# interestingLSY/swiftLLM

Measured on AMD Instinct MI355X. Metric: decode tok/s (llama3-8b bfloat16, batch 32/GPU, 1024-in/128-out; prefill tok/s alongside), higher is better.
Workload: dtype bf16

## Files before the change

swiftllm_amd/csrc/prefill_attn.hip:

```cpp
#include <stdlib.h>

#include "prefill_tile.h"

namespace swl {

struct PrefillParams {
    void *o;
    const void *q;
    const void *k;
    const void *v;
    const int *cu_seqlens;
    int num_seqs, H, KVH, num_q_blocks;
    int hpw;
    float scale_log2e;
    int64_t q_tok_stride, k_tok_stride, v_tok_stride, o_tok_stride;
};

template <typename T, int D>
__global__ __launch_bounds__(256, 2) void prefill_attn_kernel(PrefillParams p) {
    constexpr int KRS = D + 8;
    constexpr int VRS = D + 32;
    constexpr int KSTEPS = D / 16;
    constexpr int DT = D / 32;
    constexpr int CPR = D / 8;
    constexpr int RPP = 256 / CPR;
    constexpr int NPASS = kBK / RPP;
    __shared__ __attribute__((aligned(16))) T smem[kBK * KRS + kBK * VRS];
    T *const Ks = smem;
    T *const Vs = smem + kBK * KRS;

    const PrefillGrid u = PrefillGrid::decode(blockIdx.x, p.num_seqs, p.H, p.KVH, p.num_q_blocks, 1);
    if (!u.valid) return;
    const int kvh = u.kvh;
    const int head = kvh * (p.H / p.KVH) + u.hgroup;
    const int start = p.cu_seqlens[u.seq];
    const int len = p.cu_seqlens[u.seq + 1] - start;
    const int q0 = u.qb * kBQ;
    if (q0 >= len) return;

    const int tid = threadIdx.x;
    const int lane = tid & 63;
    const int wave = __builtin_amdgcn_readfirstlane(tid >> 6);
    const int l32 = lane & 31;
    const int hf = lane >> 5;
    const int q0w = q0 + wave * 32;
    const int qrow = q0w + l32;
    const float c = p.scale_log2e;

    const T *qg = static_cast<const T *>(p.q);
    const T *kg = static_cast<const T *>(p.k) + static_cast<int64_t>(kvh) * D;
    const T *vg = static_cast<const T *>(p.v) + static_cast<int64_t>(kvh) * D;

    vec8_t<T> qf[KSTEPS];
    prefill_load_q<T, D>(qf, qg, start, head, p.q_tok_stride, qrow, len, hf);

    float16_t ot[DT];
#pragma unroll
    for (int dt = 0; dt < DT; ++dt) ot[dt] = float16_t{};
    float m_run = kNegBig;
    float l_run = 0.f;

    const int srow = tid / CPR;
    const int sc = tid % CPR;
    vec8_t<T> kst[NPASS], vst[NPASS];
    const T *kp[NPASS], *vp[NPASS];
#pragma unroll
    for (int ps = 0; ps < NPASS; ++ps) {
        const int64_t tok = static_cast<int64_t>(start) + srow + ps * RPP;
        kp[ps] = kg + tok * p.k_tok_stride + sc * 8;
        vp[ps] = vg + tok * p.v_tok_stride + sc * 8;
    }
    const int64_t kstep = static_cast<int64_t>(kBK) * p.k_tok_stride, vstep = static_cast<int64_t>(kBK) * p.v_tok_stride;
    auto fetch_tile = [&](int key0) {
        if (key0 + kBK <= len) {
#pragma unroll
            for (int ps = 0; ps < NPASS; ++ps) {
                kst[ps] = load8(kp[ps]);
                vst[ps] = load8(vp[ps]);
            }
        } else {
#pragma unroll
            for (int ps = 0; ps < NPASS; ++ps) {
                vec8_t<T> kt = vec8_t<T>{}, vt = vec8_t<T>{};
                if (key0 + srow + ps * RPP < len) {
                    kt = load8(kp[ps]);
                    vt = load8(vp[ps]);
                }
                kst[ps] = kt;
                vst[ps] = vt;
            }
        }
#pragma unroll
        for (int ps = 0; ps < NPASS; ++ps) {
            kp[ps] += kstep;
            vp[ps] += vstep;
        }
    };
    auto commit_tile = [&]() {
#pragma unroll
        for (int ps = 0; ps < NPASS; ++ps) {
            const int r = srow + ps * RPP;
            *reinterpret_cast<vec8_t<T> *>(&Ks[r * KRS + sc * 8]) = kst[ps];
            *reinterpret_cast<vec8_t<T> *>(&Vs[r * VRS + sc * 8]) = vst[ps];
        }
    };

    const int kv_end = min(len, q0 + kBQ);
    const int ntiles = (kv_end + kBK - 1) / kBK;

    const int k_frag_off = l32 * KRS + hf * 8;
    const int i16 = lane & 15;
    const int v_frag_off = (4 * hf + (i16 >> 2)) * VRS + 16 * ((lane >> 4) & 1) + 4 * (i16 & 3);

    fetch_tile(0);
    for (int tile = 0; tile < ntiles; ++tile) {
        const int key0 = tile * kBK;
        __syncthreads();
        commit_tile();
        __syncthreads();
        if (tile + 1 < ntiles) fetch_tile(key0 + kBK);

        if (key0 > q0w + 31) continue;
        prefill_tile<T, D, true>(
            qf, ot, m_run, l_run, c, qrow - key0 - 4 * hf, key0 + kBK - 1 > q0w,
            [&](int t, int kk) { return *reinterpret_cast<const vec8_t<T> *>(&Ks[k_frag_off + t * 32 * KRS + kk * 16]); },
            [&](int t, int ks, int dt, int half) {
                return lds_tr_read(&Vs[v_frag_off + (t * 32 + 16 * ks + 8 * half) * VRS + dt * 32]);
            });
    }

    static_assert(4 * 32 * (D + 8) <= kBK * KRS + kBK * VRS, "the four waves' O tiles must fit the K/V tiles' LDS");
    __syncthreads();
    T *obase = static_cast<T *>(p.o) + static_cast<int64_t>(start) * p.o_tok_stride + static_cast<int64_t>(head) * D;
    prefill_store_rows<T, D, false>(ot, l_run, 1.0f, smem + wave * 32 * (D + 8), obase, p.o_tok_stride, q0w, len, lane, l32, hf);
}

__device__ __forceinline__ void dma_4_pieces(const unsigned (&off)[4], const char *base, unsigned lds) {
#pragma unroll
    for (int jj = 0; jj < 4; ++jj) {
        unsigned keep;
        asm volatile("s_mov_b32 %0, m0\n\ts_mov_b32 m0, %3\n\ts_nop 4\n\tglobal_load_lds_dwordx4 %1, %2\n\ts_mov_b32 m0, %0"
                     : "=&s"(keep) : "v"(off[jj]), "s"(base), "s"(lds + jj * 1024) : "memory");
    }
}

template <typename T>
__global__ __launch_bounds__(256, 2) void prefill_attn_dma_kernel(PrefillParams p) {
    constexpr int D = 128;
    constexpr int KSTEPS = D / 16, DT = D / 32;
    constexpr int ROWB = D * 2;
    constexpr int TILEB = kBK * ROWB;
    __shared__ __attribute__((aligned(16))) char smem[2 * 2 * TILEB];

    const int hpw = p.hpw;
    const int rows_wg = (4 / hpw) * 32;
    const PrefillGrid u = PrefillGrid::decode(blockIdx.x, p.num_seqs, p.H, p.KVH, p.num_q_blocks, hpw);
    if (!u.valid) return;
    const int kvh = u.kvh;
    const int start = p.cu_seqlens[u.seq];
    const int len = p.cu_seqlens[u.seq + 1] - start;
    const int q0 = u.qb * rows_wg;
    if (q0 >= len) return;

    const int tid = threadIdx.x;
    const int lane = tid & 63;
    const int wave = __builtin_amdgcn_readfirstlane(tid >> 6);
    const int head = kvh * (p.H / p.KVH) + u.hgroup * hpw + wave % hpw;
    const int l32 = lane & 31;
    const int hf = lane >> 5;
    const int q0w = q0 + (wave / hpw) * 32;
    const int qrow = q0w + l32;
    const float c = p.scale_log2e;

    const T *qg = static_cast<const T *>(p.q);
    vec8_t<T> qf[KSTEPS];

    float16_t ot[DT];
#pragma unroll
    for (int dt = 0; dt < DT; ++dt) ot[dt] = float16_t{};
    float m_run = kNegBig;
    float l_run = 0.f;

    const int drow = (lane >> 4);
    const int dslot = lane & 15;
    const unsigned lds0 = static_cast<unsigned>(reinterpret_cast<uintptr_t>(
        (__attribute__((address_space(3))) char *)smem));
    const int64_t kstride_b = p.k_tok_stride * 2, vstride_b = p.v_tok_stride * 2;
    unsigned koff[4], voff[4];
    auto dma_offsets = [&](int rows_valid) {
#pragma unroll
        for (int jj = 0; jj < 4; ++jj) {
            const int r = 16 * wave + 4 * jj + drow;
            const int rs = min(r, rows_valid - 1);
            koff[jj] = static_cast<unsigned>(rs * kstride_b) + static_cast<unsigned>((dslot ^ (r & 15)) * 16);
            voff[jj] = static_cast<unsigned>(rs * vstride_b) +
                       static_cast<unsigned>(((((dslot >> 2) ^ (r & 3)) << 2) | (dslot & 3)) * 16);
        }
    };
    dma_offsets(kBK);
    const char *kbase = reinterpret_cast<const char *>(static_cast<const T *>(p.k) + static_cast<int64_t>(kvh) * D) +
                        static_cast<int64_t>(start) * kstride_b;
    const char *vbase = reinterpret_cast<const char *>(static_cast<const T *>(p.v) + static_cast<int64_t>(kvh) * D) +
                        static_cast<int64_t>(start) * vstride_b;
    auto issue_tile = [&](int tile, int buf) {
        const char *kb = kbase + static_cast<int64_t>(tile) * kBK * kstride_b;
        const char *vb = vbase + static_cast<int64_t>(tile) * kBK * vstride_b;
        const unsigned ldsk = lds0 + static_cast<unsigned>(buf) * 2 * TILEB + static_cast<unsigned>(wave) * 4096;
        dma_4_pieces(koff, kb, ldsk);
        dma_4_pieces(voff, vb, ldsk + TILEB);
    };

    const int kv_end = min(len, q0 + rows_wg);
    const int ntiles = (kv_end + kBK - 1) / kBK;
    const int last_rows = kv_end - (ntiles - 1) * kBK > 0 ? min(kBK, len - (ntiles - 1) * kBK) : kBK;

    unsigned kfo[KSTEPS];
#pragma unroll
    for (int kk = 0; kk < KSTEPS; ++kk) kfo[kk] = static_cast<unsigned>(l32 * ROWB + (((2 * kk + hf) ^ (l32 & 15)) * 16));
    const int i16 = lane & 15;
    unsigned vfo[DT];
#pragma unroll
    for (int dt = 0; dt < DT; ++dt)
        vfo[dt] = static_cast<unsigned>(TILEB + (4 * hf + (i16 >> 2)) * ROWB + ((dt ^ ((i16 >> 2) & 3)) * 64) +
                                        32 * ((lane >> 4) & 1) + 8 * (i16 & 3));

    if (ntiles == 1 && last_rows < kBK) dma_offsets(last_rows);
    issue_tile(0, 0);
    {
        T *qs = reinterpret_cast<T *>(smem + 2 * TILEB) + wave * 32 * D;
        const int rsub = lane >> 4, pc = lane & 15;
        vec8_t<T> t[8];
#pragma unroll
        for (int i = 0; i < 8; ++i) {
            const int row = 4 * i + rsub;
            const bool ok = q0w + row < len;
            t[i] = load8(qg + (static_cast<int64_t>(start) + (ok ? q0w + row : 0)) * p.q_tok_stride +
                         static_cast<int64_t>(head) * D + pc * 8);
            if (!ok) t[i] = vec8_t<T>{};
        }
#pragma unroll
        for (int i = 0; i < 8; ++i) {
            const int row = 4 * i + rsub;
            *reinterpret_cast<vec8_t<T> *>(qs + row * D + ((pc ^ (row & 15)) << 3)) = t[i];
        }
#pragma unroll
        for (int kk = 0; kk < KSTEPS; ++kk)
            qf[kk] = *reinterpret_cast<const vec8_t<T> *>(qs + l32 * D + (((2 * kk + hf) ^ (l32 & 15)) << 3));
        asm volatile("s_waitcnt lgkmcnt(0)" ::: "memory");
    }
    for (int tile = 0; tile < ntiles; ++tile) {
        const int key0 = tile * kBK;
        const int buf = tile & 1;
        asm volatile("s_waitcnt vmcnt(0)" ::: "memory");
        __builtin_amdgcn_s_barrier();
        if (tile + 1 < ntiles) {
            if (tile + 2 == ntiles && last_rows < kBK) dma_offsets(last_rows);
            issue_tile(tile + 1, buf ^ 1);
        }
        if (key0 > q0w + 31) continue;
        const char *bufp = smem + buf * 2 * TILEB;
        prefill_tile<T, D, false>(
            qf, ot, m_run, l_run, c, qrow - key0 - 4 * hf, key0 + kBK - 1 > q0w,
            [&](int t, int kk) { return *reinterpret_cast<const vec8_t<T> *>(bufp + kfo[kk] + t * 32 * ROWB); },
            [&](int t, int ks, int dt, int half) {
                return lds_tr_read(reinterpret_cast<const T *>(bufp + vfo[dt] + (t * 32 + 16 * ks + 8 * half) * ROWB));
            });
    }

    static_assert(4 * 32 * (D + 8) * 2 <= 4 * TILEB, "the four waves' O tiles must fit the K/V buffers");
    __syncthreads();
    T *obase = static_cast<T *>(p.o) + static_cast<int64_t>(start) * p.o_tok_stride + static_cast<int64_t>(head) * D;
    prefill_store_rows<T, D, false>(ot, l_run, 1.0f, reinterpret_cast<T *>(smem) + wave * 32 * (D + 8), obase,
                                    p.o_tok_stride, q0w, len, lane, l32, hf);
}

}

extern "C" int swl_prefill_attn_varlen(void *o, const void *q, const void *k, const void *v,
                                       const int32_t *cu_seqlens, int32_t num_prefill_seqs,
                                       int32_t max_prefill_len, int32_t num_q_heads,
                                       int32_t num_kv_heads, int32_t head_dim, float softmax_scale,
                                       int64_t q_tok_stride, int64_t k_tok_stride,
                                       int64_t v_tok_stride, int64_t o_tok_stride, int32_t dtype,
                                       swl_stream_t stream) {
    if (num_prefill_seqs < 0 || max_prefill_len < 0) return SWL_ERR_BAD_ARG;
    if (num_prefill_seqs == 0 || max_prefill_len == 0) return SWL_OK;
    if (!o || !q || !k || !v || !cu_seqlens) return SWL_ERR_BAD_ARG;
    if (num_q_heads <= 0 || num_kv_heads <= 0 || num_q_heads % num_kv_heads != 0)
        return SWL_ERR_BAD_ARG;
    if (!(head_dim == 32 || head_dim == 64 || head_dim == 128)) return SWL_ERR_UNSUPPORTED;
    if ((q_tok_stride & 7) || (k_tok_stride & 7) || (v_tok_stride & 7) || (o_tok_stride & 7))
        return SWL_ERR_BAD_ARG;
    const int64_t q_row = static_cast<int64_t>(num_q_heads) * head_dim, kv_row = static_cast<int64_t>(num_kv_heads) * head_dim;
    if (q_tok_stride < q_row || o_tok_stride < q_row || k_tok_stride < kv_row || v_tok_stride < kv_row)
        return SWL_ERR_BAD_ARG;
    if (!swl::aligned16(q) || !swl::aligned16(k) || !swl::aligned16(v) || !swl::aligned16(o))
        return SWL_ERR_BAD_ARG;
    swl::PrefillParams p;
    p.o = o;
    p.q = q;
    p.k = k;
    p.v = v;
    p.cu_seqlens = cu_seqlens;
    p.num_seqs = num_prefill_seqs;
    p.H = num_q_heads;
    p.KVH = num_kv_heads;
    p.num_q_blocks = (max_prefill_len + swl::kBQ - 1) / swl::kBQ;
    p.scale_log2e = softmax_scale * 1.44269504088896340736f;
    p.q_tok_stride = q_tok_stride;
    p.k_tok_stride = k_tok_stride;
    p.v_tok_stride = v_tok_stride;
    p.o_tok_stride = o_tok_stride;
    p.hpw = 1;
    const int G = num_q_heads / num_kv_heads;
    dim3 grid;
    if (!swl::prefill_grid_blocks(num_prefill_seqs, num_kv_heads, G, p.num_q_blocks, &grid)) return SWL_ERR_UNSUPPORTED;
    hipStream_t s = static_cast<hipStream_t>(stream);
    static const bool use_v1 = [] { const char *e = getenv("SWL_PREFILL_ATTN"); return e && e[0] == 'v' && e[1] == '1'; }();
    const bool fits32 = static_cast<int64_t>(swl::kBK) * (k_tok_stride > v_tok_stride ? k_tok_stride : v_tok_stride) * 2 + 4096 < (1ll << 32);
    SWL_DISPATCH_DTYPE(dtype, T, {
        if (head_dim == 128 && !use_v1 && fits32) {
            static const int forced_hpw = [] { const char *e = getenv("SWL_PREFILL_HPW"); return e ? atoi(e) : 0; }();
            p.hpw = G % 2 == 0 ? 2 : 1;
            if (forced_hpw == 1 || forced_hpw == 2 || forced_hpw == 4) p.hpw = G % forced_hpw == 0 ? forced_hpw : p.hpw;
            const int rows_wg = (4 / p.hpw) * 32;
            p.num_q_blocks = (max_prefill_len + rows_wg - 1) / rows_wg;
            if (!swl::prefill_grid_blocks(num_prefill_seqs, num_kv_heads, G / p.hpw, p.num_q_blocks, &grid))
                return SWL_ERR_UNSUPPORTED;
            hipLaunchKernelGGL((swl::prefill_attn_dma_kernel<T>), grid, dim3(256), 0, s, p);
        }
        else if (head_dim == 128)
            hipLaunchKernelGGL((swl::prefill_attn_kernel<T, 128>), grid, dim3(256), 0, s, p);
        else if (head_dim == 64)
            hipLaunchKernelGGL((swl::prefill_attn_kernel<T, 64>), grid, dim3(256), 0, s, p);
        else
            hipLaunchKernelGGL((swl::prefill_attn_kernel<T, 32>), grid, dim3(256), 0, s, p);
    });
    return swl::check_launch();
}
```

swiftllm_amd/csrc/prefill_tile.h:

```cpp
#pragma once

#include "attn_mfma.h"

namespace swl {

constexpr int kBQ = 128;
constexpr int kBK = 64;

struct PrefillGrid {
    bool valid;
    int seq, kvh;
    int hgroup;
    int qb;
    static __device__ __forceinline__ PrefillGrid decode(int id, int num_seqs, int H, int KVH, int num_q_blocks, int hpw) {
        const int hgroups = H / KVH / hpw;
        const int per_unit = hgroups * num_q_blocks;
        const int xcd = id & 7;
        const int j = id >> 3;
        const int unit = xcd + 8 * (j / per_unit);
        const int inner = j % per_unit;
        return {unit < num_seqs * KVH, unit / KVH, unit % KVH, inner % hgroups, num_q_blocks - 1 - inner / hgroups};
    }
};

static inline bool prefill_grid_blocks(int num_seqs, int KVH, int hgroups, int num_q_blocks, dim3 *grid) {
    const int64_t units = static_cast<int64_t>(num_seqs) * KVH;
    const int64_t nblocks = (units + 7) / 8 * 8 * hgroups * num_q_blocks;
    if (nblocks > 0x7fffffffLL) return false;
    *grid = dim3(static_cast<unsigned>(nblocks));
    return true;
}

template <typename T, int D>
__device__ __forceinline__ void prefill_load_q(vec8_t<T> (&qf)[D / 16], const T *qg, int start, int head,
                                               int64_t q_tok_stride, int qrow, int len, int hf) {
    const bool ok = qrow < len;
    const T *qp = qg + (static_cast<int64_t>(start) + (ok ? qrow : 0)) * q_tok_stride + static_cast<int64_t>(head) * D + hf * 8;
#pragma unroll
    for (int kk = 0; kk < D / 16; ++kk) {
        vec8_t<T> t = load8(qp + kk * 16);
        if (!ok) t = vec8_t<T>{};
        qf[kk] = t;
    }
}

template <typename T, int D, bool PRIO, typename KFrag, typename VFrag>
__device__ __forceinline__ void prefill_tile(const vec8_t<T> (&qf)[D / 16], float16_t (&ot)[D / 32], float &m_run,
                                             float &l_run, float c, int dmask, bool diagonal, KFrag kfrag, VFrag vfrag) {
    constexpr int KSTEPS = D / 16, DT = D / 32;
    float16_t st[2];
    if constexpr (PRIO) __builtin_amdgcn_s_setprio(1);
#pragma unroll
    for (int t = 0; t < 2; ++t) {
        st[t] = float16_t{};
#pragma unroll
        for (int kk = 0; kk < KSTEPS; ++kk) {
            const vec8_t<T> kf = kfrag(t, kk);
            st[t] = mfma32(kf, qf[kk], st[t]);
        }
    }
    if constexpr (PRIO) __builtin_amdgcn_s_setprio(0);
    mfma_results_tie(st[0]);
    mfma_results_ready<8>(st[1]);
    if (diagonal) {
#pragma unroll
        for (int t = 0; t < 2; ++t)
#pragma unroll
            for (int r = 0; r < 16; ++r) {
                if ((r & 3) + 8 * (r >> 2) + t * 32 > dmask) st[t][r] = kNegBig;
            }
    }
    float mx = st[0][0];
#pragma unroll
    for (int t = 0; t < 2; ++t)
#pragma unroll
        for (int r = 0; r < 16; ++r) mx = fmaxf(mx, st[t][r]);
    mx = fmaxf(mx, __shfl_xor(mx, 32, 64));
    const float m_cand = fmaxf(m_run, mx * c);
    const float m_new = m_cand - m_run > kLazyMax ? m_cand : m_run;
    const float alpha = fast_exp2(m_run - m_new);
    m_run = m_new;
    float psum = 0.f;
#pragma unroll
    for (int t = 0; t < 2; ++t)
#pragma unroll
        for (int r = 0; r < 16; ++r) {
            const float pv = fast_exp2(fmaf(st[t][r], c, -m_new));
            st[t][r] = pv;
            psum += pv;
        }
    l_run = fmaf(l_run, alpha, psum);
    if (!__all(alpha == 1.0f)) {
#pragma unroll
        for (int dt = 0; dt < DT; ++dt)
#pragma unroll
            for (int r = 0; r < 16; ++r) ot[dt][r] *= alpha;
    }

    if constexpr (PRIO) __builtin_amdgcn_s_setprio(1);
#pragma unroll
    for (int t = 0; t < 2; ++t)
#pragma unroll
        for (int ks = 0; ks < 2; ++ks) {
            vec8_t<T> pb;
#pragma unroll
            for (int jj = 0; jj < 8; ++jj) pb[jj] = to_t<T>(st[t][8 * ks + jj]);
#pragma unroll
            for (int dt = 0; dt < DT; ++dt) {
                const short4_t lo = vfrag(t, ks, dt, 0);
                const short4_t hi = vfrag(t, ks, dt, 1);
                typedef short short8_t __attribute__((ext_vector_type(8)));
                const short8_t both = {lo[0], lo[1], lo[2], lo[3], hi[0], hi[1], hi[2], hi[3]};
                ot[dt] = mfma32(__builtin_bit_cast(vec8_t<T>, both), pb, ot[dt]);
            }
        }
    if constexpr (PRIO) __builtin_amdgcn_s_setprio(0);
}

template <typename T, int D, bool SCALED>
__device__ __forceinline__ void prefill_store_rows(float16_t (&ot)[D / 32], float l_run, float v_scale, T *ow, T *obase,
                                                   int64_t o_tok_stride, int q0w, int len, int lane, int l32, int hf) {
    constexpr int DT = D / 32, ORS = D + 8, CPR = D / 8;
    constexpr int RPI = 64 / CPR;
#pragma unroll
    for (int dt = 0; dt < DT; ++dt) mfma_results_tie(ot[dt]);
    mfma_results_ready<8>(ot[DT - 1]);
    const float l_tot = l_run + __shfl_xor(l_run, 32, 64);
    const float inv = 1.0f / l_tot;
#pragma unroll
    for (int dt = 0; dt < DT; ++dt)
#pragma unroll
        for (int r4 = 0; r4 < 4; ++r4) {
            typename Vec4<T>::type ov;
#pragma unroll
            for (int e = 0; e < 4; ++e) {
                float x = ot[dt][4 * r4 + e] * inv;
                if constexpr (SCALED) x *= v_scale;
                ov[e] = to_t<T>(x);
            }
            *reinterpret_cast<typename Vec4<T>::type *>(ow + l32 * ORS + dt * 32 + 8 * r4 + 4 * hf) = ov;
        }
#pragma unroll
    for (int i = 0; i < 32 / RPI; ++i) {
        const int row = i * RPI + lane / CPR, ch = lane % CPR;
        const vec8_t<T> v = *reinterpret_cast<const vec8_t<T> *>(ow + row * ORS + ch * 8);
        if (q0w + row < len) store8(obase + static_cast<int64_t>(q0w + row) * o_tok_stride + ch * 8, v);
    }
}

}
```

Measured before the change: 7667.

## Pair causal prefill q-blocks per workgroup and peel diagonal tile specializations

The DMA prefill attention kernel now gives each workgroup two q-blocks, a short one and a long one mirrored across the sequence. This balances causal work and halves the grid. K/V loading for the second pass is prefetched while the first pass finishes, and the O tile staging reuses a separately sized buffer. A PEEL variant specializes the tile routine into no-mask, low-diagonal and high-diagonal versions, skipping masking and the fully masked half tile at compile time. Both are on by default behind env vars. The change affects only prefill attention, and the metric is decode tok/s, so any effect on it would be indirect.

```diff
diff --git a/swiftllm_amd/csrc/prefill_attn.hip b/swiftllm_amd/csrc/prefill_attn.hip
--- a/swiftllm_amd/csrc/prefill_attn.hip
+++ b/swiftllm_amd/csrc/prefill_attn.hip
@@ -12,6 +12,7 @@
     const int *cu_seqlens;
     int num_seqs, H, KVH, num_q_blocks;
     int hpw;
+    int pair;
     float scale_log2e;
     int64_t q_tok_stride, k_tok_stride, v_tok_stride, o_tok_stride;
 };
@@ -144,13 +145,21 @@
     }
 }
 
-template <typename T>
+template <int N>
+struct IntC {
+    static constexpr int value = N;
+};
+
+template <typename T, bool PEEL>
 __global__ __launch_bounds__(256, 2) void prefill_attn_dma_kernel(PrefillParams p) {
     constexpr int D = 128;
     constexpr int KSTEPS = D / 16, DT = D / 32;
     constexpr int ROWB = D * 2;
     constexpr int TILEB = kBK * ROWB;
-    __shared__ __attribute__((aligned(16))) char smem[2 * 2 * TILEB];
+    constexpr int OTB = 4 * 32 * (D + 8) * 2;
+    constexpr int BUFP = OTB;
+    static_assert(2 * TILEB <= BUFP && OTB <= BUFP, "the O tiles over buffer b stay clear of buffer b ^ 1");
+    __shared__ __attribute__((aligned(16))) char smem[BUFP + 2 * TILEB];
 
     const int hpw = p.hpw;
     const int rows_wg = (4 / hpw) * 32;
@@ -159,8 +168,14 @@
     const int kvh = u.kvh;
     const int start = p.cu_seqlens[u.seq];
     const int len = p.cu_seqlens[u.seq + 1] - start;
-    const int q0 = u.qb * rows_wg;
-    if (q0 >= len) return;
+    const int n_s = (len + rows_wg - 1) / rows_wg;
+    int first = u.qb, second = u.qb;
+    if (p.pair) {
+        second = p.num_q_blocks - 1 - u.qb;
+        first = n_s - 1 - second;
+    }
+    if (first < second || first >= n_s) return;
+    const int npass = first != second ? 2 : 1;
 
     const int tid = threadIdx.x;
     const int lane = tid & 63;
@@ -168,26 +183,18 @@
     const int head = kvh * (p.H / p.KVH) + u.hgroup * hpw + wave % hpw;
     const int l32 = lane & 31;
     const int hf = lane >> 5;
-    const int q0w = q0 + (wave / hpw) * 32;
-    const int qrow = q0w + l32;
+    const int rb32 = (wave / hpw) * 32;
     const float c = p.scale_log2e;
 
     const T *qg = static_cast<const T *>(p.q);
     vec8_t<T> qf[KSTEPS];
 
-    float16_t ot[DT];
-#pragma unroll
-    for (int dt = 0; dt < DT; ++dt) ot[dt] = float16_t{};
-    float m_run = kNegBig;
-    float l_run = 0.f;
-
-    const int drow = (lane >> 4);
-    const int dslot = lane & 15;
     const unsigned lds0 = static_cast<unsigned>(reinterpret_cast<uintptr_t>(
         (__attribute__((address_space(3))) char *)smem));
     const int64_t kstride_b = p.k_tok_stride * 2, vstride_b = p.v_tok_stride * 2;
-    unsigned koff[4], voff[4];
-    auto dma_offsets = [&](int rows_valid) {
+    auto dma_offsets = [&](unsigned (&koff)[4], unsigned (&voff)[4], int ln, int rows_valid) {
+        const int drow = (ln >> 4);
+        const int dslot = ln & 15;
 #pragma unroll
         for (int jj = 0; jj < 4; ++jj) {
             const int r = 16 * wave + 4 * jj + drow;
@@ -197,22 +204,28 @@
                        static_cast<unsigned>(((((dslot >> 2) ^ (r & 3)) << 2) | (dslot & 3)) * 16);
         }
     };
-    dma_offsets(kBK);
     const char *kbase = reinterpret_cast<const char *>(static_cast<const T *>(p.k) + static_cast<int64_t>(kvh) * D) +
                         static_cast<int64_t>(start) * kstride_b;
     const char *vbase = reinterpret_cast<const char *>(static_cast<const T *>(p.v) + static_cast<int64_t>(kvh) * D) +
                         static_cast<int64_t>(start) * vstride_b;
-    auto issue_tile = [&](int tile, int buf) {
+    auto launder = [](int x) {
+        asm volatile("" : "+v"(x));
+        return x;
+    };
+    auto issue_tile = [&](const unsigned (&koff)[4], const unsigned (&voff)[4], int tile, int buf, int rows, bool fresh) {
         const char *kb = kbase + static_cast<int64_t>(tile) * kBK * kstride_b;
         const char *vb = vbase + static_cast<int64_t>(tile) * kBK * vstride_b;
-        const unsigned ldsk = lds0 + static_cast<unsigned>(buf) * 2 * TILEB + static_cast<unsigned>(wave) * 4096;
-        dma_4_pieces(koff, kb, ldsk);
-        dma_4_pieces(voff, vb, ldsk + TILEB);
+        const unsigned ldsk = lds0 + static_cast<unsigned>(buf) * BUFP + static_cast<unsigned>(wave) * 4096;
+        if (rows < kBK || fresh) {
+            unsigned ko[4], vo[4];
+            dma_offsets(ko, vo, launder(lane), rows);
+            dma_4_pieces(ko, kb, ldsk);
+            dma_4_pieces(vo, vb, ldsk + TILEB);
+        } else {
+            dma_4_pieces(koff, kb, ldsk);
+            dma_4_pieces(voff, vb, ldsk + TILEB);
+        }
     };
-
-    const int kv_end = min(len, q0 + rows_wg);
-    const int ntiles = (kv_end + kBK - 1) / kBK;
-    const int last_rows = kv_end - (ntiles - 1) * kBK > 0 ? min(kBK, len - (ntiles - 1) * kBK) : kBK;
 
     unsigned kfo[KSTEPS];
 #pragma unroll
@@ -224,10 +237,18 @@
         vfo[dt] = static_cast<unsigned>(TILEB + (4 * hf + (i16 >> 2)) * ROWB + ((dt ^ ((i16 >> 2) & 3)) * 64) +
                                         32 * ((lane >> 4) & 1) + 8 * (i16 & 3));
 
-    if (ntiles == 1 && last_rows < kBK) dma_offsets(last_rows);
-    issue_tile(0, 0);
+    auto block_tiles = [&](int qb) { return (min(len, (qb + 1) * rows_wg) + kBK - 1) / kBK; };
+    int q0 = first * rows_wg;
+    int ntiles = block_tiles(first);
+    int last_rows = min(kBK, len - (ntiles - 1) * kBK);
+
     {
-        T *qs = reinterpret_cast<T *>(smem + 2 * TILEB) + wave * 32 * D;
+        const unsigned none[4] = {};
+        issue_tile(none, none, 0, 0, ntiles == 1 ? last_rows : kBK, true);
+    }
+    {
+        const int q0w = q0 + rb32;
+        T *qs = reinterpret_cast<T *>(smem + BUFP) + wave * 32 * D;
         const int rsub = lane >> 4, pc = lane & 15;
         vec8_t<T> t[8];
 #pragma unroll
@@ -248,30 +269,91 @@
             qf[kk] = *reinterpret_cast<const vec8_t<T> *>(qs + l32 * D + (((2 * kk + hf) ^ (l32 & 15)) << 3));
         asm volatile("s_waitcnt lgkmcnt(0)" ::: "memory");
     }
-    for (int tile = 0; tile < ntiles; ++tile) {
-        const int key0 = tile * kBK;
-        const int buf = tile & 1;
+
+    vec8_t<T> qn[KSTEPS];
+    int g = 0;
+    T *const obase = static_cast<T *>(p.o) + static_cast<int64_t>(start) * p.o_tok_stride + static_cast<int64_t>(head) * D;
+#pragma nounroll
+    for (int pass = 0;; ++pass) {
+        const bool more = pass + 1 < npass;
+        const int q0w = q0 + rb32;
+        const int qrow = q0w + l32;
+        float16_t ot[DT];
+#pragma unroll
+        for (int dt = 0; dt < DT; ++dt) ot[dt] = float16_t{};
+        float m_run = kNegBig;
+        float l_run = 0.f;
+        unsigned koff[4], voff[4];
+        dma_offsets(koff, voff, launder(lane), kBK);
+
+        auto step = [&](int tile, bool fresh) {
+            asm volatile("s_waitcnt vmcnt(0)" ::: "memory");
+            __builtin_amdgcn_s_barrier();
+            if (tile + 1 < ntiles)
+                issue_tile(koff, voff, tile + 1, (g + 1) & 1, tile + 2 == ntiles ? last_rows : kBK, fresh);
+            else if (more) issue_tile(koff, voff, 0, (g + 1) & 1, kBK, fresh);
+        };
+        auto body = [&](auto diag, int tile) {
+            const int key0 = tile * kBK;
+            const char *bufp = smem + (g & 1) * BUFP;
+            prefill_tile<T, D, false, decltype(diag)::value>(
+                qf, ot, m_run, l_run, c, qrow - key0 - 4 * hf, key0 + kBK - 1 > q0w,
+                [&](int t, int kk) { return *reinterpret_cast<const vec8_t<T> *>(bufp + kfo[kk] + t * 32 * ROWB); },
+                [&](int t, int ks, int dt, int half) {
+                    return lds_tr_read(reinterpret_cast<const T *>(bufp + vfo[dt] + (t * 32 + 16 * ks + 8 * half) * ROWB));
+                });
+        };
+
+        int tile = 0;
+        if constexpr (PEEL) {
+            const int below = min(q0w / kBK, ntiles - 1);
+#pragma nounroll
+            for (; tile < below; ++tile, ++g) {
+                step(tile, false);
+                body(IntC<kDiagNone>{}, tile);
+            }
+            {
+                step(tile, false);
+                if (q0w & 32) {
+                    asm volatile("; diagonal tile, rows from key 32" ::: "memory");
+                    body(IntC<kDiagHigh>{}, tile);
+                } else {
+                    asm volatile("; diagonal tile, rows from key 0" ::: "memory");
+                    body(IntC<kDiagLow>{}, tile);
+                }
+                ++tile, ++g;
+                for (; tile < ntiles; ++tile, ++g) step(tile, true);
+            }
+        } else {
+            for (; tile < ntiles; ++tile, ++g) {
+                step(tile, false);
+                if (tile * kBK > q0w + 31) continue;
+                body(IntC<kDiagRuntime>{}, tile);
+            }
+        }
+
+        const int ln = launder(lane);
+        if (more) {
+            const T *qp = qg + (static_cast<int64_t>(start) + second * rows_wg + rb32 + (ln & 31)) * p.q_tok_stride +
+                          static_cast<int64_t>(head) * D + (ln >> 5) * 8;
+#pragma unroll
+            for (int kk = 0; kk < KSTEPS; ++kk) qn[kk] = load8(qp + kk * 16);
+        }
+        asm volatile("s_waitcnt lgkmcnt(0)" ::: "memory");
+        __builtin_amdgcn_s_barrier();
+        prefill_store_rows<T, D, false>(ot, l_run, 1.0f, reinterpret_cast<T *>(smem + ((g - 1) & 1) * 2 * TILEB) + wave * 32 * (D + 8),
+                                        obase, p.o_tok_stride, q0w, len, ln, ln & 31, ln >> 5);
+        if (!more) break;
         asm volatile("s_waitcnt vmcnt(0)" ::: "memory");
-        __builtin_amdgcn_s_barrier();
-        if (tile + 1 < ntiles) {
-            if (tile + 2 == ntiles && last_rows < kBK) dma_offsets(last_rows);
-            issue_tile(tile + 1, buf ^ 1);
-        }
-        if (key0 > q0w + 31) continue;
-        const char *bufp = smem + buf * 2 * TILEB;
-        prefill_tile<T, D, false>(
-            qf, ot, m_run, l_run, c, qrow - key0 - 4 * hf, key0 + kBK - 1 > q0w,
-            [&](int t, int kk) { return *reinterpret_cast<const vec8_t<T> *>(bufp + kfo[kk] + t * 32 * ROWB); },
-            [&](int t, int ks, int dt, int half) {
-                return lds_tr_read(reinterpret_cast<const T *>(bufp + vfo[dt] + (t * 32 + 16 * ks + 8 * half) * ROWB));
-            });
-    }
-
-    static_assert(4 * 32 * (D + 8) * 2 <= 4 * TILEB, "the four waves' O tiles must fit the K/V buffers");
-    __syncthreads();
-    T *obase = static_cast<T *>(p.o) + static_cast<int64_t>(start) * p.o_tok_stride + static_cast<int64_t>(head) * D;
-    prefill_store_rows<T, D, false>(ot, l_run, 1.0f, reinterpret_cast<T *>(smem) + wave * 32 * (D + 8), obase,
-                                    p.o_tok_stride, q0w, len, lane, l32, hf);
+#pragma unroll
+        for (int kk = 0; kk < KSTEPS; ++kk) {
+            asm volatile("" : "+v"(qn[kk]));
+            qf[kk] = qn[kk];
+        }
+        q0 = second * rows_wg;
+        ntiles = block_tiles(second);
+        last_rows = kBK;
+    }
 }
 
 }
@@ -312,6 +394,7 @@
     p.v_tok_stride = v_tok_stride;
     p.o_tok_stride = o_tok_stride;
     p.hpw = 1;
+    p.pair = 0;
     const int G = num_q_heads / num_kv_heads;
     dim3 grid;
     if (!swl::prefill_grid_blocks(num_prefill_seqs, num_kv_heads, G, p.num_q_blocks, &grid)) return SWL_ERR_UNSUPPORTED;
@@ -325,9 +408,14 @@
             if (forced_hpw == 1 || forced_hpw == 2 || forced_hpw == 4) p.hpw = G % forced_hpw == 0 ? forced_hpw : p.hpw;
             const int rows_wg = (4 / p.hpw) * 32;
             p.num_q_blocks = (max_prefill_len + rows_wg - 1) / rows_wg;
+            static const bool pair = [] { const char *e = getenv("SWL_PREFILL_PAIR"); return !(e && e[0] == '0'); }();
+            static const bool peel = [] { const char *e = getenv("SWL_PREFILL_PEEL"); return !(e && e[0] == '0'); }();
+            p.pair = pair;
+            if (pair) p.num_q_blocks = (p.num_q_blocks + 1) / 2;
             if (!swl::prefill_grid_blocks(num_prefill_seqs, num_kv_heads, G / p.hpw, p.num_q_blocks, &grid))
                 return SWL_ERR_UNSUPPORTED;
-            hipLaunchKernelGGL((swl::prefill_attn_dma_kernel<T>), grid, dim3(256), 0, s, p);
+            if (peel) hipLaunchKernelGGL((swl::prefill_attn_dma_kernel<T, true>), grid, dim3(256), 0, s, p);
+            else hipLaunchKernelGGL((swl::prefill_attn_dma_kernel<T, false>), grid, dim3(256), 0, s, p);
         }
         else if (head_dim == 128)
             hipLaunchKernelGGL((swl::prefill_attn_kernel<T, 128>), grid, dim3(256), 0, s, p);
diff --git a/swiftllm_amd/csrc/prefill_tile.h b/swiftllm_amd/csrc/prefill_tile.h
--- a/swiftllm_amd/csrc/prefill_tile.h
+++ b/swiftllm_amd/csrc/prefill_tile.h
@@ -44,14 +44,16 @@
     }
 }
 
-template <typename T, int D, bool PRIO, typename KFrag, typename VFrag>
+constexpr int kDiagRuntime = 0, kDiagNone = 1, kDiagLow = 2, kDiagHigh = 3;
+template <typename T, int D, bool PRIO, int DIAG = kDiagRuntime, typename KFrag, typename VFrag>
 __device__ __forceinline__ void prefill_tile(const vec8_t<T> (&qf)[D / 16], float16_t (&ot)[D / 32], float &m_run,
                                              float &l_run, float c, int dmask, bool diagonal, KFrag kfrag, VFrag vfrag) {
     constexpr int KSTEPS = D / 16, DT = D / 32;
-    float16_t st[2];
+    constexpr int NT = DIAG == kDiagLow ? 1 : 2;
+    float16_t st[NT];
     if constexpr (PRIO) __builtin_amdgcn_s_setprio(1);
 #pragma unroll
-    for (int t = 0; t < 2; ++t) {
+    for (int t = 0; t < NT; ++t) {
         st[t] = float16_t{};
 #pragma unroll
         for (int kk = 0; kk < KSTEPS; ++kk) {
@@ -60,11 +62,11 @@
         }
     }
     if constexpr (PRIO) __builtin_amdgcn_s_setprio(0);
-    mfma_results_tie(st[0]);
-    mfma_results_ready<8>(st[1]);
-    if (diagonal) {
+    if constexpr (NT == 2) mfma_results_tie(st[0]);
+    mfma_results_ready<8>(st[NT - 1]);
+    if (DIAG == kDiagRuntime ? diagonal : DIAG != kDiagNone) {
 #pragma unroll
-        for (int t = 0; t < 2; ++t)
+        for (int t = DIAG == kDiagHigh ? 1 : 0; t < NT; ++t)
 #pragma unroll
             for (int r = 0; r < 16; ++r) {
                 if ((r & 3) + 8 * (r >> 2) + t * 32 > dmask) st[t][r] = kNegBig;
@@ -72,7 +74,7 @@
     }
     float mx = st[0][0];
 #pragma unroll
-    for (int t = 0; t < 2; ++t)
+    for (int t = 0; t < NT; ++t)
 #pragma unroll
         for (int r = 0; r < 16; ++r) mx = fmaxf(mx, st[t][r]);
     mx = fmaxf(mx, __shfl_xor(mx, 32, 64));
@@ -82,7 +84,7 @@
     m_run = m_new;
     float psum = 0.f;
 #pragma unroll
-    for (int t = 0; t < 2; ++t)
+    for (int t = 0; t < NT; ++t)
 #pragma unroll
         for (int r = 0; r < 16; ++r) {
             const float pv = fast_exp2(fmaf(st[t][r], c, -m_new));
@@ -99,7 +101,7 @@
 
     if constexpr (PRIO) __builtin_amdgcn_s_setprio(1);
 #pragma unroll
-    for (int t = 0; t < 2; ++t)
+    for (int t = 0; t < NT; ++t)
 #pragma unroll
         for (int ks = 0; ks < 2; ++ks) {
             vec8_t<T> pb;
```

Result: no change. 7659 (-0.1%).
